# multicom-toolbox/Chromosome3D

Measured on AMD Instinct MI355X. Metric: SA-steps/sec (replica-steps/s, 20 replicas of chr1_500kb in all: 20 per GPU, weak scaling; regions of 20 steps inside the first 2172 of the schedule's 5172: MD and FIRE steps in front of the final minimisation); wall-clock per chromosome, higher is better.
Workload: dtype f32

## Files before the change

chromosome3d_amd/csrc/c3d_api.cpp:

```cpp
#include <hip/hip_runtime.h>

#include <algorithm>
#include <atomic>
#include <cmath>
#include <cstdio>
#include <cstdlib>
#include <chrono>
#include <cstring>
#include <condition_variable>
#include <map>
#include <mutex>
#include <string>
#include <thread>
#include <tuple>
#include <vector>

#include "../../include/c3d.h"
#include "c3d_host.h"
#include "c3d_internal.h"

using c3d::fail;

namespace {

#define HIP_TRY(expr)                                                                          \
    do {                                                                                       \
        hipError_t e__ = (expr);                                                               \
        if (e__ != hipSuccess)                                                                 \
            return fail(C3D_ERR_HIP, std::string(#expr) + ": " + hipGetErrorString(e__));      \
    } while (0)

template <class T>
struct DevTmp {
    T* p = nullptr;
    ~DevTmp() { if (p) (void)hipFree(p); }
};

struct Op {
    c3d::DevStep p;
    int stage;
    bool counted;
};

struct KernelRecord {
    enum Family { NONE, STEP, LBFGS_EVAL, PAIRS_SYM, STEP64, LBFGS_EVAL64, CLUSTER } family = NONE;
    c3d::StepForm step{};
    c3d::Form64 f64{};
    int pot = 0, rpw = 0, nb = 0, wl = 0;
    bool rs1 = false, late = false, tp = false;
};

inline void philox4x32(const uint32_t ctr_in[4], const uint32_t key_in[2], uint32_t out[4]) {
    uint32_t c[4] = {ctr_in[0], ctr_in[1], ctr_in[2], ctr_in[3]};
    uint32_t k[2] = {key_in[0], key_in[1]};
    for (int r = 0; r < 10; ++r) {
        const uint64_t p0 = (uint64_t)0xD2511F53u * c[0];
        const uint64_t p1 = (uint64_t)0xCD9E8D57u * c[2];
        const uint32_t n0 = (uint32_t)(p1 >> 32) ^ c[1] ^ k[0];
        const uint32_t n1 = (uint32_t)p1;
        const uint32_t n2 = (uint32_t)(p0 >> 32) ^ c[3] ^ k[1];
        const uint32_t n3 = (uint32_t)p0;
        c[0] = n0; c[1] = n1; c[2] = n2; c[3] = n3;
        k[0] += 0x9E3779B9u;
        k[1] += 0xBB67AE85u;
    }
    memcpy(out, c, sizeof(c));
}
inline double u01(uint32_t u) { return ((double)u + 0.5) * (1.0 / 4294967296.0); }
void normals4(uint64_t seed, uint32_t replica, uint32_t bead, uint32_t purpose, double g[4]) {
    const uint32_t ctr[4] = {bead, purpose, 0u, 0u};
    const uint32_t key[2] = {(uint32_t)(seed & 0xFFFFFFFFu) ^ (replica * 0x9E3779B9u), (uint32_t)(seed >> 32) + replica};
    uint32_t r[4];
    philox4x32(ctr, key, r);
    const double two_pi = 6.283185307179586476925286766559;
    double a = sqrt(-2.0 * log(u01(r[0]))), b = two_pi * u01(r[1]);
    g[0] = a * cos(b); g[1] = a * sin(b);
    a = sqrt(-2.0 * log(u01(r[2]))); b = two_pi * u01(r[3]);
    g[2] = a * cos(b); g[3] = a * sin(b);
}

}

// ... 637 lines not shown
                                       c->op_run[c->pc], c->op_skip[c->pc], (int)nops, seq << 20, c->h_tmo_dev,
                                       c->d_claim + c3d_ctx::kClaimWords * seq, c->stream);
    if (e != hipSuccess) return fail(C3D_ERR_HIP, std::string("cluster launch: ") + hipGetErrorString(e));
    if (c->event_timing) HIP_TRY(hipEventRecord(c->ev1, c->stream));
    const auto h1 = std::chrono::steady_clock::now();
    bool marked = false;
    if (c->spin_wait_us > 0 && !c->kernel_timing) {
        const unsigned mark = (seq << 20) | 1u;
        for (;;) {
            if (__atomic_load_n(&c->h_tmo[1], __ATOMIC_ACQUIRE) == mark) { marked = true; break; }
            if (__atomic_load_n(&c->h_tmo[0], __ATOMIC_RELAXED) || __atomic_load_n(&c->h_tmo[2], __ATOMIC_RELAXED)) break;
            if (std::chrono::duration<double, std::micro>(std::chrono::steady_clock::now() - h1).count() > c->spin_wait_us) break;
            __builtin_ia32_pause();
        }
    }
    if (!marked) HIP_TRY(hipStreamSynchronize(c->stream));
    else ++c->spin_completions;
    const auto h2 = std::chrono::steady_clock::now();
    c->last_host_launch_us += std::chrono::duration<double, std::micro>(h1 - h0).count();
    c->last_host_sync_us += std::chrono::duration<double, std::micro>(h2 - h1).count();
    c->ev1_recorded = true;
    ++c->cluster_launches;
    if (c->kernel_timing) {
        float kms = 0;
        HIP_TRY(hipEventElapsedTime(&kms, c->kev0, c->kev1));
        c->last_kernel_ms += kms;
    }
    if (launch_was_abandoned(c, (seq << 20) | 1u)) { *ran = false; c->ev1_recorded = false; return C3D_OK; }
    *ran = true;
    c->last_path = 2;
    KernelRecord& k = c->ran;
    k = KernelRecord();
    k.family = KernelRecord::CLUSTER;
    k.pot = c3d::device_pot(m.noe_pot); k.rpw = pl.rpw; k.nb = m.npad / 256; k.wl = m.wl; k.late = pl.late_tiles != 0; k.tp = pl.two_point;
    account_ops(c, nops);
    return C3D_OK;
}

int run_ops_segment(c3d_ctx* c, size_t nops, bool zero_w, bool lbfgs = false);

int run_ops(c3d_ctx* c, size_t nops) {
    const bool p64 = c->precision == 64;
    if (p64 ? !c->has_lbfgs : (!c->zero_weight && !c->has_two_point && !c->has_lbfgs)) return run_ops_segment(c, nops, false);
    const size_t end = c->pc + nops;
    while (c->pc < end) {
        const c3d::DevStep& p0 = c->program[c->pc].p;
        const bool z = !p64 && p0.w_rs == 0.0f, tp = !p64 && is_two_point(p0.kind), lb = is_lbfgs(p0.kind);
        size_t k = 1;
        while (c->pc + k < end) {
            const c3d::DevStep& p = c->program[c->pc + k].p;
            if ((!p64 && p.w_rs == 0.0f) != z || (!p64 && is_two_point(p.kind)) != tp || is_lbfgs(p.kind) != lb) break;
            ++k;
        }
        const int rc = run_ops_segment(c, k, z, lb);
        if (rc) return rc;
    }
    return C3D_OK;
}

int ensure_group_streams(c3d_ctx* c, int G) {
    for (int g = 1; g < G && g < c3d_ctx::kMaxGroups; ++g) {
        if (c->gstream[g]) continue;
        HIP_TRY(hipStreamCreateWithFlags(&c->gstream[g], hipStreamNonBlocking));
        HIP_TRY(hipEventCreateWithFlags(&c->gev[g], hipEventDisableTiming));
    }
    return C3D_OK;
}
// ... 1004 lines not shown
    else if (!strcmp(key, "last_path")) *value = (double)c->last_path;
    else if (!strcmp(key, "rank_prefetch_hits")) *value = (double)c->rank_prefetch_hits;
    else if (!strcmp(key, "device_rank_runs")) *value = (double)c->device_rank_runs;
    else if (!strcmp(key, "score_wide_runs")) *value = (double)c->score_wide_runs;
    else if (!strcmp(key, "compare_runs")) *value = (double)c->compare_runs;
    else if (!strcmp(key, "f64_evals")) *value = (double)c->f64_evals;
    else if (!strcmp(key, "superpose_runs")) *value = (double)c->superpose_runs;
    else if (!strcmp(key, "rmsd_table_runs")) *value = (double)c->rmsd_table_runs;
    else if (!strcmp(key, "cluster_xcd_count")) *value = (double)c->xcd_count;
    else if (!strcmp(key, "cluster_xcd_base")) *value = (double)c->xcd_base;
    else if (!strcmp(key, "cluster_ok")) *value = c->cl_ok ? 1.0 : 0.0;
    else if (!strcmp(key, "cluster_parts")) *value = c->cl_ok ? (double)c->cl_plan.parts : 0.0;
    else if (!strcmp(key, "cluster_rows_per_wave")) *value = c->cl_ok ? (double)c->cl_plan.rpw : 0.0;
    else if (!strcmp(key, "cluster_late_tiles")) *value = c->cl_ok ? (double)c->cl_plan.late_tiles : 0.0;
    else if (!strcmp(key, "cluster_compute_waves")) *value = c->cl_ok ? (double)c->cl_plan.cw : 0.0;
    else if (!strcmp(key, "cluster_helper_waves")) *value = c->cl_ok ? (double)c->cl_plan.helpers : 0.0;
    else if (!strcmp(key, "cluster_wgs_per_cu")) *value = c->cl_ok ? (double)c->cl_plan.wgs_per_cu : 0.0;
    else if (!strcmp(key, "replica_groups")) *value = (double)active_groups(c);
    else if (!strcmp(key, "embed_form")) *value = (double)c->last_embed_form;
    else if (!strcmp(key, "embed_batches")) *value = (double)c->last_embed_batches;
    else if (!strcmp(key, "units_loaded")) *value = (double)g_units.loads.load();
    else if (!strcmp(key, "units_loaded_mask")) *value = (double)g_units.loaded[c->device & (kMaxDevices - 1)].load();
    else return fail(C3D_ERR_INVALID, std::string("c3d_get_stat: unknown key ") + key);
    return C3D_OK;
}

extern "C" const char* c3d_step_kernel_name(const c3d_ctx* c) {
    static thread_local char buf[96];
    if (!c) return "";
    const KernelRecord& k = c->ran;
    auto tf = [](bool b) { return b ? "true" : "false"; };
    switch (k.family) {
        case KernelRecord::CLUSTER:
            snprintf(buf, sizeof(buf), "c3d::k_cluster%s<%d, %d, %d, %d, %s>", k.tp ? "_tp" : "", k.pot, k.rpw, k.nb, k.wl, tf(k.late));
            break;
        case KernelRecord::STEP64:
        case KernelRecord::LBFGS_EVAL64: {
            const char* kernel = k.family == KernelRecord::STEP64 ? "k64_step" : "k64_lbfgs_eval";
            if (k.f64.chunk) snprintf(buf, sizeof(buf), "c3d::%s_chunked<%d, %s, %s, %d>", kernel, k.f64.pot, tf(k.f64.gen), tf(k.f64.fold), k.f64.chunk);
            else snprintf(buf, sizeof(buf), "c3d::%s<%d, %s, %s>", kernel, k.f64.pot, tf(k.f64.gen), tf(k.f64.fold));
            break;
        }
        case KernelRecord::PAIRS_SYM: snprintf(buf, sizeof(buf), "c3d::k_pairs_sym<%d, %s, false>", k.pot, tf(k.rs1)); break;
        case KernelRecord::STEP:
        case KernelRecord::LBFGS_EVAL: {
            const char* kernel = k.family == KernelRecord::STEP ? "k_step" : "k_lbfgs_eval";
            if (k.step.chunk) {
                if (k.step.wide) snprintf(buf, sizeof(buf), "c3d::%s_chunked<4, false, 4, 16, true, %d>", kernel, k.step.chunk);
                else snprintf(buf, sizeof(buf), "c3d::%s_chunked<%d, %s, %d, 8, false, %d>", kernel, k.step.pot, tf(k.step.gen), k.step.rpw, k.step.chunk);
            } else if (k.step.wide) snprintf(buf, sizeof(buf), "c3d::%s<4, false, 4, false, 16, true>", kernel);
            else snprintf(buf, sizeof(buf), "c3d::%s<%d, %s, %d, %s, 8, false>", kernel, k.step.pot, tf(k.step.gen), k.step.rpw, tf(k.step.nc));
            break;
        }
        default: return "";
    }
    return buf;
}

extern "C" int c3d_eval(c3d_ctx* c, float w_all, float w_vdw, float repel_s, float* F, double* e) {
    if (!c || !c->have_replicas) return fail(C3D_ERR_INVALID, "c3d_eval: bad state");
    C3D_ENTRY(c, 0u);
    const c3d::DevModel m = dev_model(c);
    const c3d::DevStep p = dev_step(c, 3, 0.0f, w_all, w_vdw, repel_s, 0.0f);
    if (F) {
        hipError_t err = c3d::launch_eval_forces(m, p, c->buf, c->parity, c->d_feval, c3d::general_step(m, p), c->eval_rpw,
                                                 c3d::column_chunk_for(m, c->column_chunk), c->stream);
        if (err != hipSuccess) return fail(C3D_ERR_HIP, std::string("eval launch: ") + hipGetErrorString(err));
// ... 463 lines not shown
    int rc = c3d_get_energies(c, e.data());
    if (rc) return rc;
    std::vector<int32_t> idx(c->nrep);
    for (int r = 0; r < c->nrep; ++r) idx[r] = r;
    std::stable_sort(idx.begin(), idx.end(), [&](int a, int b) { return (long long)e[3 * a] < (long long)e[3 * b]; });
    for (int r = 0; r < c->nrep; ++r) rank[r] = idx[r];
    return C3D_OK;
}

extern "C" int c3d_debug_tear16(c3d_ctx* c, int iterations, unsigned long long* unit_reads, unsigned long long* torn, unsigned long long* fresh) {
    if (!c || iterations < 1 || iterations > (1 << 24)) return fail(C3D_ERR_INVALID, "c3d_debug_tear16: bad arguments");
    C3D_ENTRY(c, unit_bit(UNIT_CLUSTER_BASE));
    DevTmp<unsigned char> buf;
    DevTmp<unsigned> stop;
    DevTmp<unsigned long long> stats;
    HIP_TRY(hipMalloc(&buf.p, 1024 * 16));
    HIP_TRY(hipMalloc(&stop.p, sizeof(unsigned)));
    HIP_TRY(hipMalloc(&stats.p, 3 * sizeof(unsigned long long)));
    HIP_TRY(hipMemsetAsync(buf.p, 0, 1024 * 16, c->stream));
    HIP_TRY(hipMemsetAsync(stop.p, 0, sizeof(unsigned), c->stream));
    HIP_TRY(hipMemsetAsync(stats.p, 0, 3 * sizeof(unsigned long long), c->stream));
    hipError_t e = c3d::launch_tear16(c->num_cus, buf.p, stop.p, stats.p, iterations, c->stream);
    if (e != hipSuccess) return fail(C3D_ERR_HIP, std::string("tear16 launch: ") + hipGetErrorString(e));
    unsigned long long h[3] = {0, 0, 0};
    HIP_TRY(hipMemcpyAsync(h, stats.p, sizeof h, hipMemcpyDeviceToHost, c->stream));
    HIP_TRY(hipStreamSynchronize(c->stream));
    if (unit_reads) *unit_reads = h[0];
    if (torn) *torn = h[1];
    if (fresh) *fresh = h[2];
    return C3D_OK;
}

#ifdef C3D_STAMPS
namespace c3d { hipError_t read_stamps(unsigned long long* out); hipError_t read_cluster_stamps(unsigned long long* out); hipError_t read_cluster_pstamps(unsigned long long* out); }
extern "C" int c3d_debug_cluster_pstamps(unsigned long long* out) {
    hipError_t e = c3d::read_cluster_pstamps(out);
    return e == hipSuccess ? C3D_OK : C3D_ERR_HIP;
}
extern "C" int c3d_debug_cluster_stamps(unsigned long long* out) {
    hipError_t e = c3d::read_cluster_stamps(out);
    return e == hipSuccess ? C3D_OK : C3D_ERR_HIP;
}
extern "C" int c3d_debug_stamps(unsigned long long* out) {
    hipError_t e = c3d::read_stamps(out);
    return e == hipSuccess ? C3D_OK : C3D_ERR_HIP;
}
#endif
```

chromosome3d_amd/csrc/c3d_cluster.hip:

```cpp
#include <hip/hip_ext.h>
#include <atomic>
#include <type_traits>
#include <cstdio>
#include <cstdlib>

#include "c3d_step_core.h"

namespace c3d {

typedef unsigned u32x4 __attribute__((ext_vector_type(4)));
constexpr int kClMaxThreads = 1024;

#ifdef C3D_STAMPS
__device__ unsigned long long g_cstamps[64][8];
__device__ unsigned long long g_pstamps[8];
#define CSTAMP(k) do { if (stamper) g_cstamps[s & 63][k] = __builtin_amdgcn_s_memrealtime(); } while (0)
#define CSTAMP_C(k) do { if (cstamper) g_cstamps[s & 63][k] = __builtin_amdgcn_s_memrealtime(); } while (0)
#else
#define CSTAMP(k) do { } while (0)
#define CSTAMP_C(k) do { } while (0)
#endif

template <int POT, int RPW, int NB, int WL, bool LATE, bool TWO>
__device__ __forceinline__ void cluster_body(
    const float* __restrict__ tgt, unsigned* __restrict__ claim, const StepRun* __restrict__ runs, const int P, const int CW, const int NH,
    const int static_place, const int nbeads, const int run0, const int skip0, const int nsteps,
    const unsigned tag_base, u32x4* __restrict__ rec, volatile unsigned* __restrict__ timeout, const unsigned expected,
    const AnnealIO& io, const DevModel& m, const DevFire& fp) {
    constexpr int NPAD = 256 * NB;
    constexpr int MAXT = NPAD / 8;
    constexpr int KUMAX = NB > 2 ? 3 : 2;
    extern __shared__ __attribute__((aligned(16))) float smem[];
    float* xs = smem;
    float* ys = smem + NPAD;
    float* zs = smem + 2 * NPAD;
    float* ps = smem + 3 * NPAD;
    float* fbuf = ps + 4 * MAXT;
    float* cbuf = fbuf + 3 * 64;
    float* lbuf = cbuf + 3 * 64;
    float* lcon = lbuf + 3 * 64;
    float* dump = lcon + 3 * 4 * 2 * 64;
    int* s_slot = reinterpret_cast<int*>(dump + 4);
#ifdef C3D_STAMPS
    const unsigned long long t_entry = __builtin_amdgcn_s_memrealtime();
#endif
    const int tid = threadIdx.x, lane = tid & 63, wave = tid >> 6;
    const int nthreads = (CW + NH) * 64;
    const int RW = CW * RPW;

    const int xcc = (int)(__builtin_amdgcn_s_getreg((3 << 11) | 20) & 0x7);
    const int sp_mode = static_place & 0xff, xcd0 = (static_place >> 8) & 0xff, nxcd = (static_place >> 16) & 0xff;
    int slot;
    if (sp_mode) {
        const unsigned off = ((unsigned)xcc - blockIdx.x + (sp_mode == 2 && blockIdx.x == 0 ? 1u : 0u)) & 7u;
        if (tid == 0) atomicOr(&claim[9], 1u << off);
        slot = (int)(blockIdx.x >> 3);
// ... 2 lines not shown
        __syncthreads();
        slot = *s_slot;
    }
    const int lxcd = xcc - xcd0;
    const int lrep = lxcd + nxcd * (slot / P), part = slot % P;
#ifdef C3D_STAMPS
    const unsigned long long t_placed = __builtin_amdgcn_s_memrealtime();
#endif
    const bool is_compute = wave >= NH, is_h0 = wave == 0;
    const int cwave = wave - NH;
    const int wg_row0 = part * RW;
    const int row0 = wg_row0 + cwave * RPW;
    const StepRun first_run = runs[run0];
    float4 traw[RPW][NB];
#pragma unroll
    for (int r = 0; r < RPW; ++r)
#pragma unroll
        for (int jb = 0; jb < NB; ++jb) {
            float4 t = make_float4(0, 0, 0, 0);
            if (is_compute) {
                const float* trow = tgt + (size_t)min(row0 + r, nbeads - 1) * NPAD + 256 * jb;
                if (jb < NB - 1 || WL == 4) t = *reinterpret_cast<const float4*>(trow + 4 * lane);
                else if constexpr (WL == 3) {
                    struct F3 { float a, b, c; };
                    const F3 q = *reinterpret_cast<const F3*>(trow + 3 * lane);
                    t = make_float4(q.a, q.b, q.c, 0.0f);
                } else if constexpr (WL == 2) {
                    const float2 q = *reinterpret_cast<const float2*>(trow + 2 * lane);
                    t = make_float4(q.x, q.y, 0.0f, 0.0f);
                } else t = make_float4(trow[lane], 0.0f, 0.0f, 0.0f);
            }
            traw[r][jb] = t;
        }
    if (lxcd < 0 || lxcd >= nxcd || lrep >= m.nrep_g) return;
    const int rep = m.rep_base + lrep;
    const bool solo = P == 1;
    if (!is_compute) __builtin_amdgcn_s_setprio(3);

    const size_t roff = (size_t)rep * 3 * NPAD;
    const int hrow = wg_row0 + lane;
    const bool hfin = is_h0 && lane < RW && hrow < m.n;
#define C3D_HROW_INDEX const size_t ix = roff + hrow, iy = ix + NPAD, iz = iy + NPAD
    constexpr int rec_stride = NPAD + NPAD / 4;
    constexpr int KT = (MAXT + 63) / 64;
    constexpr bool late = LATE;
    const int gthreads = late ? nthreads - 64 : nthreads;
    const int gtid = late ? tid - 64 : tid;
    const int units = late ? m.n : m.n + 2 * m.ntiles;
    const int ku = (units + gthreads - 1) / gthreads;
    const auto rsrc = __builtin_amdgcn_make_buffer_rsrc(rec, 0, (int)(sizeof(u32x4) * 2 * m.nrep_g * rec_stride), 0x00020000);

    float vcx = 0.0f, vcy = 0.0f, vcz = 0.0f;
    FireState st;
    float4 cin[2], pin4 = make_float4(0, 0, 0, 0);
    {
        const float* xin = io.xin;
        const float* pin = io.pin;
        const float* vin = io.vin;
#pragma unroll
        for (int k = 0; k < 2; ++k) {
            const int b = 4 * (tid + k * nthreads);
            cin[k] = b < 3 * NPAD ? *reinterpret_cast<const float4*>(xin + roff + b) : make_float4(0, 0, 0, 0);
        }
        if (tid < m.ntiles) pin4 = reinterpret_cast<const float4*>(pin)[(size_t)rep * m.ntiles + tid];
        if (hfin) { C3D_HROW_INDEX; vcx = vin[ix]; vcy = vin[iy]; vcz = vin[iz]; }
        st = io.sin[rep];
    }
    float* const lc = lcon + (size_t)((wave >= 1 && wave <= 3) ? wave - 1 : 0) * (4 * 2 * 64);
    if (!is_compute && !is_h0 && wave <= 3 && m.nleft > 0) {
        for (int q = 0; q < 4; ++q) {
            const int k = 8 * (wave - 1) + 8 * (NH - 1) * q + (lane >> 3), c = lane & 7;
            float b = 0.0f, a = 0.0f;
            if (k < RW && c < m.nleft && wg_row0 + k < m.n) {
                const float t = tgt[(size_t)(wg_row0 + k) * NPAD + m.jl0 + c];
                b = t * m.inv_rs;
                a = t > 0.0f ? m.inv_rs : 0.0f;
            }
            lc[(2 * q) * 64 + lane] = b; lc[(2 * q + 1) * 64 + lane] = a;
        }
    }
#pragma unroll
    for (int k = 0; k < 2; ++k) {
        const int b = 4 * (tid + k * nthreads);
        if (b < 3 * NPAD) *reinterpret_cast<float4*>(smem + b) = cin[k];
    }
    if (tid < m.ntiles) reinterpret_cast<float4*>(ps)[tid] = pin4;
    if (tid < 3 * 64) lbuf[tid] = 0.0f;
#ifdef C3D_STAMPS
    asm volatile("s_waitcnt lgkmcnt(0)" ::: "memory");
    const unsigned long long t_coords = __builtin_amdgcn_s_memrealtime();
#endif
    constexpr bool PK = POT == 4;
    float4 tv[PK ? 1 : RPW][NB];
    PairConsts2<PK ? RPW : 1, NB> pc;
    float4* const mw = reinterpret_cast<float4*>(dump + 8) + (size_t)(is_compute ? cwave : 0) * (RPW * NB * 64);
    if constexpr (PK) {
        pair_consts2_build<RPW, NB>(m, traw, is_compute, lane, pc, mw);
    } else {
        DevStep p0{};
#pragma unroll
        for (int r = 0; r < RPW; ++r)
#pragma unroll
            for (int jb = 0; jb < NB; ++jb) {
                tv[r][jb] = pair_b<false>(m, traw[r][jb]);
                if (is_compute) mw[(r * NB + jb) * 64 + lane] = pair_a<false>(m, p0, traw[r][jb]);
            }
    }
#ifdef C3D_STAMPS
    asm volatile("s_waitcnt vmcnt(0) lgkmcnt(0)" ::: "memory");
    const unsigned long long t_targets = __builtin_amdgcn_s_memrealtime();
#endif
    int gsrc[KUMAX], gda[KUMAX], gdb[KUMAX], gdc[KUMAX];
    const int dump_off = (int)(dump - smem);
// ... 25 lines not shown
    for (int run = run0;; ++run) {
      if (run != run0) cur = runs[run];
      const DevStep p = cur.p;
      const int count = cur.count;
      const bool needs_partials = p.kind == 0 || p.kind == 1 || p.kind == 2 || (TWO && p.kind == 5);
      for (int it = run == run0 ? skip0 : 0; it < count; ++it, ++s) {
#ifdef C3D_STAMPS
        if (cstamper && s == 0) g_pstamps[7] = __builtin_amdgcn_s_memrealtime();
#endif
        __syncthreads();
        CSTAMP(0);
#ifdef C3D_STAMPS
        if (stamper && s == 0) g_pstamps[2] = __builtin_amdgcn_s_memrealtime();
#endif
        CSTAMP_C(6);

        float hx0 = 0.0f, hy0 = 0.0f, hz0 = 0.0f;
        StepScalars sc;
        sc.lam = 1.0f; sc.cmx = sc.cmy = sc.cmz = 0.0f; sc.keep = 0.0f; sc.mix = 0.0f;
        if constexpr (ROLE == 0) {
            if (p.kind != 4) {
                float Fx, Fy, Fz;
                if constexpr (PK) tile_pair_sums_pk<RPW, NB, WL>(m, p, pc, mw, xs, ys, zs, row0, lane, Fx, Fy, Fz);
                else tile_pair_sums_reg<POT, RPW, NB, WL, 1>(m, p, tv, mw, xs, ys, zs, row0, lane, Fx, Fy, Fz);
                if (lane < RPW) {
                    const int k = cwave * RPW + lane;
                    fbuf[k] = Fx; fbuf[64 + k] = Fy; fbuf[128 + k] = Fz;
                }
                CSTAMP_C(7);
            }
        } else if constexpr (ROLE == 1) {
            if (p.kind != 2 && !(TWO && p.kind == 5)) { st.dt = fp.dt_start; st.alpha = fp.alpha_start; st.npos = 0; st.pad = 0; }
            float4 psum = make_float4(0, 0, 0, 0);
            if (needs_partials) {
                if (late && !solo && s > 0) {
                    const unsigned tagp = tag_base + (unsigned)s;
                    const int basep = ((s & 1) * m.nrep_g + lrep) * rec_stride + NPAD;
                    u32x4 a[KT], b[KT];
                    unsigned spins = 0;
                    for (;;) {
                        bool ok = true;
                        asm volatile("" ::: "memory");
#pragma unroll
                        for (int k = 0; k < KT; ++k) {
                            const int t = min(lane + 64 * k, m.ntiles - 1);
                            a[k] = __builtin_amdgcn_raw_buffer_load_b128(rsrc, (basep + 2 * t) * 16, 0, 16);
                            b[k] = __builtin_amdgcn_raw_buffer_load_b128(rsrc, (basep + 2 * t + 1) * 16, 0, 16);
                        }
#pragma unroll
                        for (int k = 0; k < KT; ++k) ok &= a[k].x == tagp && b[k].x == tagp;
                        if (__all(ok)) break;
                        __builtin_amdgcn_s_sleep(1);
                        ++spins;
                        if (spins > (1u << 18) || ((spins & 1023u) == 0 && *timeout != 0u)) {
                            if (lane == 0) *timeout = 1u;
                            return;
                        }
                    }
#pragma unroll
                    for (int k = 0; k < KT; ++k)
                        if (lane + 64 * k < m.ntiles)
                            reinterpret_cast<float4*>(ps)[lane + 64 * k] = make_float4(__uint_as_float(a[k].y), __uint_as_float(a[k].z), __uint_as_float(a[k].w), __uint_as_float(b[k].y));
                }
                for (int t = lane; t < m.ntiles; t += 64) {
                    const float4 q = reinterpret_cast<const float4*>(ps)[t];
                    psum.x += q.x; psum.y += q.y; psum.z += q.z; psum.w += q.w;
                }
                psum = wave_sum4(psum);
                psum.x = __uint_as_float(__builtin_amdgcn_readfirstlane(__float_as_uint(psum.x)));
                psum.y = __uint_as_float(__builtin_amdgcn_readfirstlane(__float_as_uint(psum.y)));
                psum.z = __uint_as_float(__builtin_amdgcn_readfirstlane(__float_as_uint(psum.z)));
                psum.w = __uint_as_float(__builtin_amdgcn_readfirstlane(__float_as_uint(psum.w)));
            }
            sc = step_scalars<TWO>(m, p, fp, psum, st);
            if (lane < RW && hrow < NPAD) { hx0 = xs[hrow]; hy0 = ys[hrow]; hz0 = zs[hrow]; }
            CSTAMP(1);
        } else if (p.kind != 4) {
            for (int cb = 16 * (wave - 1); cb < RW; cb += 16 * (NH - 1)) {
                const int k = cb + (lane >> 2);
                float cx, cy, cz;
// ... 108 lines not shown
        }
        {
            if (last) return;
            if (solo) continue;
            __builtin_amdgcn_s_barrier();
            u32x4 v[KUMAX];
            unsigned spins = 0;
            for (;;) {
                bool ok = true;
                asm volatile("" ::: "memory");
#pragma unroll
                for (int k = 0; k < KUMAX; ++k)
                    if (k < ku) v[k] = __builtin_amdgcn_raw_buffer_load_b128(rsrc, (base + gsrc[k]) * 16, 0, 16);
#pragma unroll
                for (int k = 0; k < KUMAX; ++k)
                    if (k < ku) ok &= v[k].x == tag;
                if (__all(ok)) break;
                __builtin_amdgcn_s_sleep(1);
                ++spins;
                if (spins > (1u << 18) || ((spins & 1023u) == 0 && *timeout != 0u)) {
                    if (lane == 0) *timeout = 1u;
                    return;
                }
            }
#pragma unroll
            for (int k = 0; k < KUMAX; ++k)
                if (k < ku) { smem[gda[k]] = __uint_as_float(v[k].y); smem[gdb[k]] = __uint_as_float(v[k].z); smem[gdc[k]] = __uint_as_float(v[k].w); }
        }
      }
    }
    };
    if (is_compute) role_loop(std::integral_constant<int, 0>{});
    else if (is_h0) role_loop(std::integral_constant<int, 1>{});
    else role_loop(std::integral_constant<int, 2>{});
}

#define C3D_CLUSTER_ARGS                                                                                                                  \
    const float* __restrict__ tgt, unsigned* __restrict__ claim, const StepRun* __restrict__ runs, const int P, const int CW, const int NH, \
    const int static_place, const int nbeads, const int run0, const int skip0, const int nsteps, const unsigned tag_base,                 \
    u32x4* __restrict__ rec, volatile unsigned* __restrict__ timeout, const unsigned expected, const AnnealIO io, const DevModel m, const DevFire fp
#define C3D_CLUSTER_PASS tgt, claim, runs, P, CW, NH, static_place, nbeads, run0, skip0, nsteps, tag_base, rec, timeout, expected, io, m, fp
template <int POT, int RPW, int NB, int WL, bool LATE>
__global__ __launch_bounds__(kClMaxThreads) void k_cluster(C3D_CLUSTER_ARGS) { cluster_body<POT, RPW, NB, WL, LATE, false>(C3D_CLUSTER_PASS); }
template <int POT, int RPW, int NB, int WL, bool LATE>
__global__ __launch_bounds__(kClMaxThreads) void k_cluster_tp(C3D_CLUSTER_ARGS) { cluster_body<POT, RPW, NB, WL, LATE, true>(C3D_CLUSTER_PASS); }
#undef C3D_CLUSTER_ARGS
#undef C3D_CLUSTER_PASS

constexpr bool cluster_late_ok(int pot, int rpw, int nb, int wl) { return pot >= 3 && rpw * (4 * (nb - 1) + wl) >= 6; }
#ifndef C3D_CLUSTER_POT
#ifdef C3D_STAMPS
hipError_t read_cluster_stamps(unsigned long long* out) { return hipMemcpyFromSymbol(out, HIP_SYMBOL(g_cstamps), sizeof(unsigned long long) * 64 * 8); }
hipError_t read_cluster_pstamps(unsigned long long* out) { return hipMemcpyFromSymbol(out, HIP_SYMBOL(g_pstamps), sizeof(unsigned long long) * 8); }
#endif

__global__ __launch_bounds__(kClMaxThreads) void k_tear16(u32x4* buf, unsigned* stop, unsigned long long* stats, int iters) {
    const auto rsrc = __builtin_amdgcn_make_buffer_rsrc(buf, 0, kClMaxThreads * 16, 0x00020000);
    const int tid = threadIdx.x;
    if (blockIdx.x == 0) {
        for (int i = 1; i <= iters; ++i) {
            u32x4 v; v.x = v.y = v.z = v.w = (unsigned)i;
            __builtin_amdgcn_raw_buffer_store_b128(v, rsrc, tid * 16, 0, 0);
        }
        __threadfence();
        if (tid == 0) atomicExch(stop, 1u);
        return;
    }
    const auto ssrc = __builtin_amdgcn_make_buffer_rsrc(stop, 0, 4, 0x00020000);
    unsigned long long reads = 0, torn = 0, fresh = 0;
    unsigned lastv = 0;
    for (unsigned guard = 0; guard < (1u << 26); ++guard) {
        asm volatile("" ::: "memory");
        const u32x4 v = __builtin_amdgcn_raw_buffer_load_b128(rsrc, tid * 16, 0, 16);
        ++reads;
        if (!(v.x == v.y && v.y == v.z && v.z == v.w)) ++torn;
        if (v.x != lastv) { ++fresh; lastv = v.x; }
        if ((reads & 255) == 0 && __builtin_amdgcn_raw_buffer_load_b32(ssrc, 0, 0, 16) != 0u) break;
    }
    atomicAdd(&stats[0], reads); atomicAdd(&stats[1], torn); atomicAdd(&stats[2], fresh);
}
hipError_t launch_tear16(int num_cus, void* buf, unsigned* stop, unsigned long long* stats, int iters, hipStream_t s) {
    hipLaunchKernelGGL(k_tear16, dim3(num_cus), dim3(kClMaxThreads), 0, s, reinterpret_cast<u32x4*>(buf), stop, stats, iters);
    return hipGetLastError();
}


bool cluster_plan(const DevModel& m, int num_cus, int num_xcc, int forced_geom, int forced_late, int xcd_count, ClusterPlan* plan) {
    if (m.npad > 1024 || num_xcc != 8 || num_cus < 8 || num_cus % 8) return false;
    const int cus_per_xcd = num_cus / 8;
    if (xcd_count < 1 || xcd_count > 8) return false;
    const int per_xcd = (m.nrep_g + xcd_count - 1) / xcd_count;
    const int nb = m.npad / 256;
    static const int geoms[][4] = {{8, 1, 4, 1}, {8, 2, 4, 1}, {12, 2, 4, 1}, {8, 4, 4, 1}, {10, 4, 4, 1}, {12, 4, 4, 1}, {8, 3, 4, 1},
                                   {4, 2, 4, 1}, {4, 4, 4, 1}, {6, 4, 4, 1}};
    double best = 1e30;
    bool found = false;
    const int fcw = forced_geom / 100, frpw = forced_geom / 10 % 10, fnh = forced_geom % 10;
    for (const auto& g : geoms) {
        const int cw = g[0], rpw = g[1], nh = g[2], wpc = g[3], rw = cw * rpw;
        if (fcw && (cw != fcw || rpw != frpw || nh != fnh)) continue;
        if (rw % 8 || rw > 64) continue;
        if (rpw * nb > 8) continue;
        if (m.noe_pot < 3 && (m.wl != 4 || m.nleft != 0)) continue;
        if (m.nleft > 0 && (nh != 4 || (rw + 8 * (nh - 1) - 1) / (8 * (nh - 1)) > 4)) continue;
        const int P = (m.n + rw - 1) / rw;
        if (per_xcd * P > cus_per_xcd * wpc) continue;
        const int threads = (cw + nh) * 64;
        const int kumax = nb > 2 ? 3 : 2;
        const int late = P > 1 && forced_late != 0 && cluster_late_ok(m.noe_pot, rpw, nb, m.wl) &&
                         (m.noe_pot != 4 || ((cw + 3) / 4) * rpw * (4 * (nb - 1) + m.wl) >= 12);
        if ((late ? m.n : m.n + 2 * ((m.n + 7) / 8)) > (late ? threads - 64 : threads) * kumax) continue;
        size_t lds = sizeof(float) * (3 * m.npad + 4 * (m.npad / 8) + 9 * 64 + 24 * 64 + 16) + (size_t)cw * rpw * nb * 64 * 16;
        if (wpc == 1) { if (lds < 84 * 1024) lds = 84 * 1024; }
        else if (lds > 78 * 1024 || threads > 512) continue;
        const int wps = (cw * wpc + 3) / 4;
        const double per_slot = m.noe_pot == 4 ? (rpw / 2) * 22.0 + (rpw & 1) * 19.0 : rpw * 15.0;
        const double valu = (wps == 1 ? 1.6 : (wps == 2 ? 1.15 : 1.0)) * wps * ((4 * (nb - 1) + m.wl) * per_slot + 60.0);
        const double serial = 200.0 + (P > 1 ? 140.0 + 0.92 * m.n : 0.0);
        const double cost = wpc == 1 ? valu + serial : (valu > serial ? valu + 0.35 * serial : 0.5 * valu + serial);
        if (cost < best) {
            best = cost; found = true;
            plan->rpw = rpw; plan->cw = cw; plan->helpers = nh; plan->wgs_per_cu = wpc; plan->parts = P; plan->per_xcd = per_xcd;
            plan->grid = num_cus * wpc; plan->threads = threads; plan->units = 2 * rw; plan->device = 0; plan->lds = lds;
            plan->expected = (unsigned)(m.nrep_g * P);
            plan->late_tiles = late;
            plan->xcd_count = xcd_count;
        }
    }
    return found;
}

size_t cluster_record_bytes(const DevModel& m, const ClusterPlan& pl) { (void)pl; return (size_t)2 * m.nrep_g * (m.npad + m.npad / 4) * 16; }

#endif

template <int POT, int RPW, int NB, int WL, bool LATE>
static hipError_t cluster_go(const DevModel& m, const DevFire& fp, const ClusterPlan& pl, const AnnealIO& io, const float* tgt, void* rec,
                             const StepRun* runs, int run0, int skip0, int nsteps, unsigned tag_base, unsigned* timeout, unsigned* claim,
                             hipStream_t s) {
#if defined(C3D_CLUSTER_TP)
    constexpr bool kHasLean = false, kHasTp = true;
#elif defined(C3D_CLUSTER_POT)
    constexpr bool kHasLean = true, kHasTp = false;
#else
    constexpr bool kHasLean = true, kHasTp = true;
#endif
    const int tp = pl.two_point ? 1 : 0;
    if ((tp && !kHasTp) || (!tp && !kHasLean)) return hipErrorInvalidValue;
    const int sp = (pl.static_place & 0xff) | ((pl.xcd_base & 0xff) << 8) | ((pl.xcd_count & 0xff) << 16);
#define C3D_CL_LAUNCH(K)                                                                                                                              \
    do {                                                                                                                                              \
        if (pl.t0 && pl.t1)                                                                                                                           \
            hipExtLaunchKernelGGL((K<POT, RPW, NB, WL, LATE>), dim3(pl.grid), dim3(pl.threads), pl.lds, s, pl.t0, pl.t1, 0, tgt, claim, runs,          \
                                  pl.parts, pl.cw, pl.helpers, sp, m.n, run0, skip0, nsteps, tag_base, reinterpret_cast<u32x4*>(rec), timeout, pl.expected, io, m, fp); \
        else                                                                                                                                          \
            hipLaunchKernelGGL((K<POT, RPW, NB, WL, LATE>), dim3(pl.grid), dim3(pl.threads), pl.lds, s, tgt, claim, runs, pl.parts, pl.cw, pl.helpers, \
                               sp, m.n, run0, skip0, nsteps, tag_base, reinterpret_cast<u32x4*>(rec), timeout, pl.expected, io, m, fp);                \
    } while (0)
    if constexpr (kHasTp) { if (tp) C3D_CL_LAUNCH(k_cluster_tp); }
    if constexpr (kHasLean) { if (!tp) C3D_CL_LAUNCH(k_cluster); }
#undef C3D_CL_LAUNCH
    return hipGetLastError();
}
template <int POT, class F>
static void for_each_cluster_form(F&& f) {
    auto widths = [&](auto R, auto B) {
        auto w = [&](auto W) {
            f(R, B, W, bool_c<false>{});
            if constexpr (cluster_late_ok(POT, R, B, W)) f(R, B, W, bool_c<true>{});
        };
        w(int_c<4>{});
        if constexpr (POT >= 3) { w(int_c<3>{}); w(int_c<2>{}); w(int_c<1>{}); }
    };
    widths(int_c<1>{}, int_c<1>{}); widths(int_c<1>{}, int_c<2>{}); widths(int_c<1>{}, int_c<3>{}); widths(int_c<1>{}, int_c<4>{});
    widths(int_c<2>{}, int_c<1>{}); widths(int_c<2>{}, int_c<2>{}); widths(int_c<2>{}, int_c<3>{}); widths(int_c<2>{}, int_c<4>{});
    widths(int_c<3>{}, int_c<1>{}); widths(int_c<3>{}, int_c<2>{});
    widths(int_c<4>{}, int_c<1>{}); widths(int_c<4>{}, int_c<2>{});
}
template <int POT>
static hipError_t cluster_geom(const DevModel& m, const DevFire& fp, const ClusterPlan& pl, const AnnealIO& io, const float* tgt, void* rec,
                               const StepRun* runs, int run0, int skip0, int nsteps, unsigned tag_base, unsigned* timeout, unsigned* claim,
                               hipStream_t s) {
    hipError_t e = hipErrorInvalidValue;
    for_each_cluster_form<POT>([&](auto R, auto B, auto W, auto L) {
        if (pl.rpw == R && m.npad == 256 * B && m.wl == W && (pl.late_tiles != 0) == L)
            e = cluster_go<POT, R, B, W, L>(m, fp, pl, io, tgt, rec, runs, run0, skip0, nsteps, tag_base, timeout, claim, s);
    });
    return e;
}

template <int POT, bool TP>
static hipError_t cluster_prepare_unit() {
    hipError_t e = hipSuccess;
    for_each_cluster_form<POT>([&](auto R, auto B, auto W, auto L) {
        const void* k;
        if constexpr (TP) k = reinterpret_cast<const void*>(&k_cluster_tp<POT, R, B, W, L>);
        else k = reinterpret_cast<const void*>(&k_cluster<POT, R, B, W, L>);
        if (e == hipSuccess) e = hipFuncSetAttribute(k, hipFuncAttributeMaxDynamicSharedMemorySize, 160 * 1024);
    });
    return e;
}

#define C3D_CL_CAT2(a, b) a##b
#define C3D_CL_CAT(a, b) C3D_CL_CAT2(a, b)
#if defined(C3D_CLUSTER_POT) && defined(C3D_CLUSTER_TP)
hipError_t C3D_CL_CAT(launch_cluster_tp_pot, C3D_CLUSTER_POT)(const DevModel& m, const DevFire& fp, const ClusterPlan& pl, const AnnealIO& io, const float* tgt, void* rec,
                          const StepRun* runs, int run0, int skip0, int nsteps, unsigned tag_base, unsigned* timeout, unsigned* claim,
                          hipStream_t s) {
    return cluster_geom<C3D_CLUSTER_POT>(m, fp, pl, io, tgt, rec, runs, run0, skip0, nsteps, tag_base, timeout, claim, s);
}
hipError_t C3D_CL_CAT(preload_cluster_tp_pot, C3D_CLUSTER_POT)() { return cluster_prepare_unit<C3D_CLUSTER_POT, true>(); }
#elif defined(C3D_CLUSTER_POT)
hipError_t C3D_CL_CAT(launch_cluster_pot, C3D_CLUSTER_POT)(const DevModel& m, const DevFire& fp, const ClusterPlan& pl, const AnnealIO& io, const float* tgt, void* rec,
                          const StepRun* runs, int run0, int skip0, int nsteps, unsigned tag_base, unsigned* timeout, unsigned* claim,
                          hipStream_t s) {
    return cluster_geom<C3D_CLUSTER_POT>(m, fp, pl, io, tgt, rec, runs, run0, skip0, nsteps, tag_base, timeout, claim, s);
}
hipError_t C3D_CL_CAT(preload_cluster_pot, C3D_CLUSTER_POT)() { return cluster_prepare_unit<C3D_CLUSTER_POT, false>(); }
#else
using ClusterLaunch = hipError_t(const DevModel& m, const DevFire& fp, const ClusterPlan& pl, const AnnealIO& io, const float* tgt, void* rec,
                                 const StepRun* runs, int run0, int skip0, int nsteps, unsigned tag_base, unsigned* timeout, unsigned* claim,
                                 hipStream_t s);
#if defined(C3D_CLUSTER_SPLIT)
ClusterLaunch launch_cluster_pot0, launch_cluster_pot1, launch_cluster_pot2, launch_cluster_pot3, launch_cluster_pot4;
ClusterLaunch launch_cluster_tp_pot0, launch_cluster_tp_pot1, launch_cluster_tp_pot2, launch_cluster_tp_pot3, launch_cluster_tp_pot4;
hipError_t preload_cluster_pot0(), preload_cluster_pot1(), preload_cluster_pot2(), preload_cluster_pot3(), preload_cluster_pot4();
hipError_t preload_cluster_tp_pot0(), preload_cluster_tp_pot1(), preload_cluster_tp_pot2(), preload_cluster_tp_pot3(), preload_cluster_tp_pot4();
static ClusterLaunch* const kClusterLaunch[2][5] = {{launch_cluster_pot0, launch_cluster_pot1, launch_cluster_pot2, launch_cluster_pot3, launch_cluster_pot4},
                                                    {launch_cluster_tp_pot0, launch_cluster_tp_pot1, launch_cluster_tp_pot2, launch_cluster_tp_pot3, launch_cluster_tp_pot4}};
static hipError_t (*const kClusterPreload[2][5])() = {{preload_cluster_pot0, preload_cluster_pot1, preload_cluster_pot2, preload_cluster_pot3, preload_cluster_pot4},
// ... 36 lines not shown
```

Baseline: 4.680 million.

## Add single-helper cluster kernel variant with three workgroups per CU

Adds a k_cluster1 kernel family where only one helper wave exists. That helper takes over the leftover-column and chain terms that role-2 helpers used to compute, and it issues the partials buffer loads before doing that work so they overlap. The planner gains a geometry with 4 compute waves, rpw 4, 1 helper and 3 workgroups per CU, with tighter LDS and thread limits. However, the planner skips wpc==3 unless a geometry is forced, so this path likely does not run by default. Debug CU-id stamping is also added.

```diff
diff --git a/chromosome3d_amd/csrc/c3d_api.cpp b/chromosome3d_amd/csrc/c3d_api.cpp
--- a/chromosome3d_amd/csrc/c3d_api.cpp
+++ b/chromosome3d_amd/csrc/c3d_api.cpp
@@ -47,7 +47,7 @@
     c3d::StepForm step{};
     c3d::Form64 f64{};
     int pot = 0, rpw = 0, nb = 0, wl = 0;
-    bool rs1 = false, late = false, tp = false;
+    bool rs1 = false, late = false, tp = false, one = false;
 };
 
 inline void philox4x32(const uint32_t ctr_in[4], const uint32_t key_in[2], uint32_t out[4]) {
@@ -751,7 +751,7 @@
     KernelRecord& k = c->ran;
     k = KernelRecord();
     k.family = KernelRecord::CLUSTER;
-    k.pot = c3d::device_pot(m.noe_pot); k.rpw = pl.rpw; k.nb = m.npad / 256; k.wl = m.wl; k.late = pl.late_tiles != 0; k.tp = pl.two_point;
+    k.pot = c3d::device_pot(m.noe_pot); k.rpw = pl.rpw; k.nb = m.npad / 256; k.wl = m.wl; k.late = pl.late_tiles != 0; k.tp = pl.two_point; k.one = pl.helpers == 1;
     account_ops(c, nops);
     return C3D_OK;
 }
@@ -1822,7 +1822,7 @@
     auto tf = [](bool b) { return b ? "true" : "false"; };
     switch (k.family) {
         case KernelRecord::CLUSTER:
-            snprintf(buf, sizeof(buf), "c3d::k_cluster%s<%d, %d, %d, %d, %s>", k.tp ? "_tp" : "", k.pot, k.rpw, k.nb, k.wl, tf(k.late));
+            snprintf(buf, sizeof(buf), "c3d::k_cluster%s%s<%d, %d, %d, %d, %s>", k.one ? "1" : "", k.tp ? "_tp" : "", k.pot, k.rpw, k.nb, k.wl, tf(k.late));
             break;
         case KernelRecord::STEP64:
         case KernelRecord::LBFGS_EVAL64: {
@@ -2352,7 +2352,11 @@
 }
 
 #ifdef C3D_STAMPS
-namespace c3d { hipError_t read_stamps(unsigned long long* out); hipError_t read_cluster_stamps(unsigned long long* out); hipError_t read_cluster_pstamps(unsigned long long* out); }
+namespace c3d { hipError_t read_stamps(unsigned long long* out); hipError_t read_cluster_stamps(unsigned long long* out); hipError_t read_cluster_pstamps(unsigned long long* out); hipError_t read_cluster_cuids(unsigned* out); }
+extern "C" int c3d_debug_cluster_cuids(unsigned* out) {
+    hipError_t e = c3d::read_cluster_cuids(out);
+    return e == hipSuccess ? C3D_OK : C3D_ERR_HIP;
+}
 extern "C" int c3d_debug_cluster_pstamps(unsigned long long* out) {
     hipError_t e = c3d::read_cluster_pstamps(out);
     return e == hipSuccess ? C3D_OK : C3D_ERR_HIP;
diff --git a/chromosome3d_amd/csrc/c3d_cluster.hip b/chromosome3d_amd/csrc/c3d_cluster.hip
--- a/chromosome3d_amd/csrc/c3d_cluster.hip
+++ b/chromosome3d_amd/csrc/c3d_cluster.hip
@@ -14,6 +14,7 @@
 #ifdef C3D_STAMPS
 __device__ unsigned long long g_cstamps[64][8];
 __device__ unsigned long long g_pstamps[8];
+__device__ unsigned g_cuids[1024];
 #define CSTAMP(k) do { if (stamper) g_cstamps[s & 63][k] = __builtin_amdgcn_s_memrealtime(); } while (0)
 #define CSTAMP_C(k) do { if (cstamper) g_cstamps[s & 63][k] = __builtin_amdgcn_s_memrealtime(); } while (0)
 #else
@@ -21,7 +22,7 @@
 #define CSTAMP_C(k) do { } while (0)
 #endif
 
-template <int POT, int RPW, int NB, int WL, bool LATE, bool TWO>
+template <int POT, int RPW, int NB, int WL, bool LATE, bool TWO, bool ONE>
 __device__ __forceinline__ void cluster_body(
     const float* __restrict__ tgt, unsigned* __restrict__ claim, const StepRun* __restrict__ runs, const int P, const int CW, const int NH,
     const int static_place, const int nbeads, const int run0, const int skip0, const int nsteps,
@@ -90,6 +91,12 @@
             }
             traw[r][jb] = t;
         }
+#ifdef C3D_STAMPS
+    if (tid == 0 && blockIdx.x < 1024) {
+        const bool idle = lxcd < 0 || lxcd >= nxcd || lrep >= m.nrep_g;
+        g_cuids[blockIdx.x] = idle ? 0u : 0x80000000u | (unsigned)lrep << 20 | (unsigned)xcc << 16 | (__builtin_amdgcn_s_getreg((15 << 11) | 4) & 0xffffu);
+    }
+#endif
     if (lxcd < 0 || lxcd >= nxcd || lrep >= m.nrep_g) return;
     const int rep = m.rep_base + lrep;
     const bool solo = P == 1;
@@ -137,6 +144,20 @@
             lc[(2 * q) * 64 + lane] = b; lc[(2 * q + 1) * 64 + lane] = a;
         }
     }
+    if constexpr (ONE) {
+        if (is_h0 && m.nleft > 0) {
+            for (int q = 0; q < 4; ++q) {
+                const int k = 8 * q + (lane >> 3), c = lane & 7;
+                float b = 0.0f, a = 0.0f;
+                if (k < RW && c < m.nleft && wg_row0 + k < m.n) {
+                    const float t = tgt[(size_t)(wg_row0 + k) * NPAD + m.jl0 + c];
+                    b = t * m.inv_rs;
+                    a = t > 0.0f ? m.inv_rs : 0.0f;
+                }
+                lc[(2 * q) * 64 + lane] = b; lc[(2 * q + 1) * 64 + lane] = a;
+            }
+        }
+    }
 #pragma unroll
     for (int k = 0; k < 2; ++k) {
         const int b = 4 * (tid + k * nthreads);
@@ -228,20 +249,58 @@
         } else if constexpr (ROLE == 1) {
             if (p.kind != 2 && !(TWO && p.kind == 5)) { st.dt = fp.dt_start; st.alpha = fp.alpha_start; st.npos = 0; st.pad = 0; }
             float4 psum = make_float4(0, 0, 0, 0);
+            u32x4 a1[ONE ? KT : 1], b1[ONE ? KT : 1];
+            if constexpr (ONE) {
+                if (needs_partials && late && !solo && s > 0) {
+                    const int basep = ((s & 1) * m.nrep_g + lrep) * rec_stride + NPAD;
+                    asm volatile("" ::: "memory");
+#pragma unroll
+                    for (int k = 0; k < KT; ++k) {
+                        const int t = min(lane + 64 * k, m.ntiles - 1);
+                        a1[k] = __builtin_amdgcn_raw_buffer_load_b128(rsrc, (basep + 2 * t) * 16, 0, 16);
+                        b1[k] = __builtin_amdgcn_raw_buffer_load_b128(rsrc, (basep + 2 * t + 1) * 16, 0, 16);
+                    }
+                }
+                if (p.kind != 4) {
+                    {
+                        const int k = lane >> 2;
+                        float cx, cy, cz;
+                        chain_term(m, p, xs, ys, zs, wg_row0 + k, lane & 3, k < RW, cx, cy, cz);
+                        cx = quad_chain_sum(cx); cy = quad_chain_sum(cy); cz = quad_chain_sum(cz);
+                        if ((lane & 3) == 0 && k < RW) { cbuf[k] = cx; cbuf[64 + k] = cy; cbuf[128 + k] = cz; }
+                    }
+                    if (m.nleft > 0) {
+                        const PairK kk = pair_k(m, p);
+                        for (int q = 0; 8 * q < RW; ++q) {
+                            const int k = 8 * q + (lane >> 3), c = lane & 7;
+                            const bool active = k < RW && c < m.nleft && wg_row0 + k < m.n;
+                            float lx, ly, lz;
+                            leftover_terms<POT, false>(m, p, kk, xs, ys, zs, min(wg_row0 + k, m.n - 1), c, active, lc[(2 * q) * 64 + lane], lc[(2 * q + 1) * 64 + lane], lx, ly, lz);
+                            if (c == 0 && k < RW) { lbuf[k] = lx; lbuf[64 + k] = ly; lbuf[128 + k] = lz; }
+                        }
+                    }
+                }
+            }
             if (needs_partials) {
                 if (late && !solo && s > 0) {
                     const unsigned tagp = tag_base + (unsigned)s;
                     const int basep = ((s & 1) * m.nrep_g + lrep) * rec_stride + NPAD;
                     u32x4 a[KT], b[KT];
                     unsigned spins = 0;
+                    if constexpr (ONE) {
+#pragma unroll
+                        for (int k = 0; k < KT; ++k) { a[k] = a1[k]; b[k] = b1[k]; }
+                    }
                     for (;;) {
                         bool ok = true;
+                        if (!ONE || spins > 0) {
                         asm volatile("" ::: "memory");
 #pragma unroll
                         for (int k = 0; k < KT; ++k) {
                             const int t = min(lane + 64 * k, m.ntiles - 1);
                             a[k] = __builtin_amdgcn_raw_buffer_load_b128(rsrc, (basep + 2 * t) * 16, 0, 16);
                             b[k] = __builtin_amdgcn_raw_buffer_load_b128(rsrc, (basep + 2 * t + 1) * 16, 0, 16);
+                        }
                         }
 #pragma unroll
                         for (int k = 0; k < KT; ++k) ok &= a[k].x == tagp && b[k].x == tagp;
@@ -416,7 +475,7 @@
     };
     if (is_compute) role_loop(std::integral_constant<int, 0>{});
     else if (is_h0) role_loop(std::integral_constant<int, 1>{});
-    else role_loop(std::integral_constant<int, 2>{});
+    else if constexpr (!ONE) role_loop(std::integral_constant<int, 2>{});
 }
 
 #define C3D_CLUSTER_ARGS                                                                                                                  \
@@ -425,9 +484,13 @@
     u32x4* __restrict__ rec, volatile unsigned* __restrict__ timeout, const unsigned expected, const AnnealIO io, const DevModel m, const DevFire fp
 #define C3D_CLUSTER_PASS tgt, claim, runs, P, CW, NH, static_place, nbeads, run0, skip0, nsteps, tag_base, rec, timeout, expected, io, m, fp
 template <int POT, int RPW, int NB, int WL, bool LATE>
-__global__ __launch_bounds__(kClMaxThreads) void k_cluster(C3D_CLUSTER_ARGS) { cluster_body<POT, RPW, NB, WL, LATE, false>(C3D_CLUSTER_PASS); }
+__global__ __launch_bounds__(kClMaxThreads) void k_cluster(C3D_CLUSTER_ARGS) { cluster_body<POT, RPW, NB, WL, LATE, false, false>(C3D_CLUSTER_PASS); }
 template <int POT, int RPW, int NB, int WL, bool LATE>
-__global__ __launch_bounds__(kClMaxThreads) void k_cluster_tp(C3D_CLUSTER_ARGS) { cluster_body<POT, RPW, NB, WL, LATE, true>(C3D_CLUSTER_PASS); }
+__global__ __launch_bounds__(kClMaxThreads) void k_cluster_tp(C3D_CLUSTER_ARGS) { cluster_body<POT, RPW, NB, WL, LATE, true, false>(C3D_CLUSTER_PASS); }
+template <int POT, int RPW, int NB, int WL, bool LATE>
+__global__ __launch_bounds__(kClMaxThreads) void k_cluster1(C3D_CLUSTER_ARGS) { cluster_body<POT, RPW, NB, WL, LATE, false, true>(C3D_CLUSTER_PASS); }
+template <int POT, int RPW, int NB, int WL, bool LATE>
+__global__ __launch_bounds__(kClMaxThreads) void k_cluster1_tp(C3D_CLUSTER_ARGS) { cluster_body<POT, RPW, NB, WL, LATE, true, true>(C3D_CLUSTER_PASS); }
 #undef C3D_CLUSTER_ARGS
 #undef C3D_CLUSTER_PASS
 
@@ -436,6 +499,7 @@
 #ifdef C3D_STAMPS
 hipError_t read_cluster_stamps(unsigned long long* out) { return hipMemcpyFromSymbol(out, HIP_SYMBOL(g_cstamps), sizeof(unsigned long long) * 64 * 8); }
 hipError_t read_cluster_pstamps(unsigned long long* out) { return hipMemcpyFromSymbol(out, HIP_SYMBOL(g_pstamps), sizeof(unsigned long long) * 8); }
+hipError_t read_cluster_cuids(unsigned* out) { return hipMemcpyFromSymbol(out, HIP_SYMBOL(g_cuids), sizeof(unsigned) * 1024); }
 #endif
 
 __global__ __launch_bounds__(kClMaxThreads) void k_tear16(u32x4* buf, unsigned* stop, unsigned long long* stats, int iters) {
@@ -476,7 +540,7 @@
     const int per_xcd = (m.nrep_g + xcd_count - 1) / xcd_count;
     const int nb = m.npad / 256;
     static const int geoms[][4] = {{8, 1, 4, 1}, {8, 2, 4, 1}, {12, 2, 4, 1}, {8, 4, 4, 1}, {10, 4, 4, 1}, {12, 4, 4, 1}, {8, 3, 4, 1},
-                                   {4, 2, 4, 1}, {4, 4, 4, 1}, {6, 4, 4, 1}};
+                                   {4, 2, 4, 1}, {4, 4, 4, 1}, {6, 4, 4, 1}, {4, 4, 1, 3}};
     double best = 1e30;
     bool found = false;
     const int fcw = forced_geom / 100, frpw = forced_geom / 10 % 10, fnh = forced_geom % 10;
@@ -486,7 +550,9 @@
         if (rw % 8 || rw > 64) continue;
         if (rpw * nb > 8) continue;
         if (m.noe_pot < 3 && (m.wl != 4 || m.nleft != 0)) continue;
-        if (m.nleft > 0 && (nh != 4 || (rw + 8 * (nh - 1) - 1) / (8 * (nh - 1)) > 4)) continue;
+        if (wpc == 3 && !fcw) continue;
+        if (nh == 1 && (m.noe_pot < 3 || nb > 2 || rpw != 4)) continue;
+        if (m.nleft > 0 && nh == 1 ? rw > 32 : m.nleft > 0 && (nh != 4 || (rw + 8 * (nh - 1) - 1) / (8 * (nh - 1)) > 4)) continue;
         const int P = (m.n + rw - 1) / rw;
         if (per_xcd * P > cus_per_xcd * wpc) continue;
         const int threads = (cw + nh) * 64;
@@ -496,7 +562,8 @@
         if ((late ? m.n : m.n + 2 * ((m.n + 7) / 8)) > (late ? threads - 64 : threads) * kumax) continue;
         size_t lds = sizeof(float) * (3 * m.npad + 4 * (m.npad / 8) + 9 * 64 + 24 * 64 + 16) + (size_t)cw * rpw * nb * 64 * 16;
         if (wpc == 1) { if (lds < 84 * 1024) lds = 84 * 1024; }
-        else if (lds > 78 * 1024 || threads > 512) continue;
+        else if (wpc == 2) { if (lds > 78 * 1024 || threads > 512) continue; }
+        else if (lds > 52 * 1024 || threads > 320) continue;
         const int wps = (cw * wpc + 3) / 4;
         const double per_slot = m.noe_pot == 4 ? (rpw / 2) * 22.0 + (rpw & 1) * 19.0 : rpw * 15.0;
         const double valu = (wps == 1 ? 1.6 : (wps == 2 ? 1.15 : 1.0)) * wps * ((4 * (nb - 1) + m.wl) * per_slot + 60.0);
@@ -518,7 +585,7 @@
 
 #endif
 
-template <int POT, int RPW, int NB, int WL, bool LATE>
+template <int POT, int RPW, int NB, int WL, bool LATE, bool ONE = false>
 static hipError_t cluster_go(const DevModel& m, const DevFire& fp, const ClusterPlan& pl, const AnnealIO& io, const float* tgt, void* rec,
                              const StepRun* runs, int run0, int skip0, int nsteps, unsigned tag_base, unsigned* timeout, unsigned* claim,
                              hipStream_t s) {
@@ -541,8 +608,13 @@
             hipLaunchKernelGGL((K<POT, RPW, NB, WL, LATE>), dim3(pl.grid), dim3(pl.threads), pl.lds, s, tgt, claim, runs, pl.parts, pl.cw, pl.helpers, \
                                sp, m.n, run0, skip0, nsteps, tag_base, reinterpret_cast<u32x4*>(rec), timeout, pl.expected, io, m, fp);                \
     } while (0)
-    if constexpr (kHasTp) { if (tp) C3D_CL_LAUNCH(k_cluster_tp); }
-    if constexpr (kHasLean) { if (!tp) C3D_CL_LAUNCH(k_cluster); }
+    if constexpr (ONE) {
+        if constexpr (kHasTp) { if (tp) C3D_CL_LAUNCH(k_cluster1_tp); }
+        if constexpr (kHasLean) { if (!tp) C3D_CL_LAUNCH(k_cluster1); }
+    } else {
+        if constexpr (kHasTp) { if (tp) C3D_CL_LAUNCH(k_cluster_tp); }
+        if constexpr (kHasLean) { if (!tp) C3D_CL_LAUNCH(k_cluster); }
+    }
 #undef C3D_CL_LAUNCH
     return hipGetLastError();
 }
@@ -561,11 +633,31 @@
     widths(int_c<3>{}, int_c<1>{}); widths(int_c<3>{}, int_c<2>{});
     widths(int_c<4>{}, int_c<1>{}); widths(int_c<4>{}, int_c<2>{});
 }
+template <int POT, class F>
+static void for_each_cluster_one_form(F&& f) {
+    if constexpr (POT >= 3) {
+        auto widths = [&](auto B) {
+            auto w = [&](auto W) {
+                f(int_c<4>{}, B, W, bool_c<false>{});
+                if constexpr (cluster_late_ok(POT, 4, B, W)) f(int_c<4>{}, B, W, bool_c<true>{});
+            };
+            w(int_c<4>{}); w(int_c<3>{}); w(int_c<2>{}); w(int_c<1>{});
+        };
+        widths(int_c<1>{}); widths(int_c<2>{});
+    }
+}
 template <int POT>
 static hipError_t cluster_geom(const DevModel& m, const DevFire& fp, const ClusterPlan& pl, const AnnealIO& io, const float* tgt, void* rec,
                                const StepRun* runs, int run0, int skip0, int nsteps, unsigned tag_base, unsigned* timeout, unsigned* claim,
                                hipStream_t s) {
     hipError_t e = hipErrorInvalidValue;
+    if (pl.helpers == 1) {
+        for_each_cluster_one_form<POT>([&](auto R, auto B, auto W, auto L) {
+            if (pl.rpw == R && m.npad == 256 * B && m.wl == W && (pl.late_tiles != 0) == L)
+                e = cluster_go<POT, R, B, W, L, true>(m, fp, pl, io, tgt, rec, runs, run0, skip0, nsteps, tag_base, timeout, claim, s);
+        });
+        return e;
+    }
     for_each_cluster_form<POT>([&](auto R, auto B, auto W, auto L) {
         if (pl.rpw == R && m.npad == 256 * B && m.wl == W && (pl.late_tiles != 0) == L)
             e = cluster_go<POT, R, B, W, L>(m, fp, pl, io, tgt, rec, runs, run0, skip0, nsteps, tag_base, timeout, claim, s);
@@ -580,6 +672,12 @@
         const void* k;
         if constexpr (TP) k = reinterpret_cast<const void*>(&k_cluster_tp<POT, R, B, W, L>);
         else k = reinterpret_cast<const void*>(&k_cluster<POT, R, B, W, L>);
+        if (e == hipSuccess) e = hipFuncSetAttribute(k, hipFuncAttributeMaxDynamicSharedMemorySize, 160 * 1024);
+    });
+    for_each_cluster_one_form<POT>([&](auto R, auto B, auto W, auto L) {
+        const void* k;
+        if constexpr (TP) k = reinterpret_cast<const void*>(&k_cluster1_tp<POT, R, B, W, L>);
+        else k = reinterpret_cast<const void*>(&k_cluster1<POT, R, B, W, L>);
         if (e == hipSuccess) e = hipFuncSetAttribute(k, hipFuncAttributeMaxDynamicSharedMemorySize, 160 * 1024);
     });
     return e;
```

Measured after the change: 4.457 million. 4.8% lower.
